# wenet-e2e/wesep

Hardware: AMD Instinct MI355X
Metric: utterances/sec (4 s, 16 kHz, 2-spk) fwd+bwd, pBSRNN (higher is better)
Workload: dtype bf16x3+fp16x2+fp16x1 split products (+fp8 lo terms), fp32 accumulate; 1 GPU; pBSRNN FiLM multi-fuse, 6 repeats, feature_dim 128, fixed 256-d embeddings; fwd + SI-SDR + bwd + per-tensor clip + Adam-L2; bf16x3 (x-projections, projections, d(hcat), BN / mask GEMMs) + fp16x2 (recurrent products of all four recurrence kernels, d(xn)) + fp16x1 (LSTM weight gradients); 2-byte saved gates / d(gates); fp32 accumulate; BPTT kernels: W_hh as fp16 hi + block-scaled FP8 lo; the lo term; rows_per_gpu=32, global_rows=32, samples_per_row=64000, parallelism=dp1

## Files before the change

wesep_amd/csrc/gemm_blk.hip:

```cpp
#include <stdlib.h>

#include <type_traits>

#include "common.h"

typedef __bf16 bf16x8 __attribute__((ext_vector_type(8)));
typedef unsigned int u32x4 __attribute__((ext_vector_type(4)));
typedef unsigned int u32x2 __attribute__((ext_vector_type(2)));
typedef float f32x2 __attribute__((ext_vector_type(2)));
typedef _Float16 f16x8 __attribute__((ext_vector_type(8)));
typedef _Float16 f16x2 __attribute__((ext_vector_type(2)));
typedef int i32x4 __attribute__((ext_vector_type(4)));
typedef int v8i __attribute__((ext_vector_type(8)));
typedef __fp16 h16x2 __attribute__((ext_vector_type(2)));

__device__ __forceinline__ f32x16 mfma32(bf16x8 a, bf16x8 b, f32x16 c) {
  return __builtin_amdgcn_mfma_f32_32x32x16_bf16(a, b, c, 0, 0, 0);
}

__device__ __forceinline__ void split8(const float* v, bf16x8& hi, bf16x8& lo) {
#pragma unroll
  for (int j = 0; j < 8; ++j) {
    hi[j] = (__bf16)v[j];
    lo[j] = (__bf16)(v[j] - (float)hi[j]);
// ... 365 lines not shown
    const int sc = __builtin_amdgcn_readfirstlane(sc_n);
    v8i a8;
#pragma unroll
    for (int hs = 0; hs < HS; ++hs) {
    acell ac[2 * KH];
#pragma unroll
    for (int q = 0; q < 2 * KH; ++q) ac[q] = an[q];
    if (hs == 0 && st + 1 < nstage) {
      wstage(st + 1, cur ^ 1);
      if constexpr (A16 == 3) sc_n = wsc[st + 1];
    }
    if (hs + 1 < HS) load_a(st, hs + 1);
    else if (st + 1 < nstage) load_a(st + 1, 0);
#pragma unroll
    for (int ksl = 0; ksl < KH; ++ksl) {
      const int ks = hs * KH + ksl;
      bf16x8 ah, al;
      if constexpr (A16 == 1) {
        const u32x2 c0 = __builtin_bit_cast(u32x2, ac[2 * ksl]), c1 = __builtin_bit_cast(u32x2, ac[2 * ksl + 1]);
        ah = __builtin_bit_cast(bf16x8, u32x4{c0[0], c0[1], c1[0], c1[1]});
      } else if constexpr (A16 == 3) {
        const u32x2 c0 = __builtin_bit_cast(u32x2, ac[2 * ksl]), c1 = __builtin_bit_cast(u32x2, ac[2 * ksl + 1]);
        const f16x8 a16 = __builtin_bit_cast(f16x8, u32x4{c0[0], c0[1], c1[0], c1[1]});
        typedef short s16x2 __attribute__((ext_vector_type(2)));
#pragma unroll
        for (int h2 = 0; h2 < 2; ++h2) {
          s16x2 c = {0, 0};
          c = __builtin_amdgcn_cvt_scalef32_pk_fp8_f16(c, f16x2{a16[4 * h2], a16[4 * h2 + 1]}, 256.f, false);
          c = __builtin_amdgcn_cvt_scalef32_pk_fp8_f16(c, f16x2{a16[4 * h2 + 2], a16[4 * h2 + 3]}, 256.f, true);
          a8[2 * ks + h2] = __builtin_bit_cast(int, c);
        }
        const u32x4* wt = &wl[cur][ks * 256 + lane];
#pragma unroll
        for (int nt = 0; nt < 4; ++nt)
          acc[nt] = __builtin_amdgcn_mfma_f32_32x32x16_f16(a16, __builtin_bit_cast(f16x8, wt[nt * 64]), acc[nt], 0, 0, 0);
        if (ks == 3) {
          const u32x4* w8 = &wl[cur][1024 + lane];
          auto frag = [&](int nt) {
            return __builtin_shufflevector(__builtin_bit_cast(i32x4, w8[(2 * nt) * 64]), __builtin_bit_cast(i32x4, w8[(2 * nt + 1) * 64]),
                                           0, 1, 2, 3, 4, 5, 6, 7);
          };
          acc[0] = __builtin_amdgcn_mfma_scale_f32_32x32x64_f8f6f4(a8, frag(0), acc[0], 0, 0, 0, 127 + 8, 0, sc);
          acc[1] = __builtin_amdgcn_mfma_scale_f32_32x32x64_f8f6f4(a8, frag(1), acc[1], 0, 0, 0, 127 + 8, 1, sc);
          acc[2] = __builtin_amdgcn_mfma_scale_f32_32x32x64_f8f6f4(a8, frag(2), acc[2], 0, 0, 0, 127 + 8, 2, sc);
          acc[3] = __builtin_amdgcn_mfma_scale_f32_32x32x64_f8f6f4(a8, frag(3), acc[3], 0, 0, 0, 127 + 8, 3, sc);
        }
        continue;
      } else if constexpr (A16 == 2) {
        const u32x2 c0 = __builtin_bit_cast(u32x2, ac[2 * ksl]), c1 = __builtin_bit_cast(u32x2, ac[2 * ksl + 1]);
        const f16x8 a16 = __builtin_bit_cast(f16x8, u32x4{c0[0], c0[1], c1[0], c1[1]});
        const u32x4* wt = &wl[cur][ks * 512 + lane];
#pragma unroll
        for (int nt = 0; nt < 4; ++nt) {
          acc[nt] = __builtin_amdgcn_mfma_f32_32x32x16_f16(a16, __builtin_bit_cast(f16x8, wt[(nt * 2) * 64]), acc[nt], 0, 0, 0);
          acc[nt] = __builtin_amdgcn_mfma_f32_32x32x16_f16(a16, __builtin_bit_cast(f16x8, wt[(nt * 2 + 1) * 64]), acc[nt], 0, 0, 0);
        }
        continue;
      } else {
        unpack8(__builtin_bit_cast(u32x4, ac[2 * ksl]), __builtin_bit_cast(u32x4, ac[2 * ksl + 1]), ah, al);
        if (p.a16_out && active) {
          unsigned short* o16 = reinterpret_cast<unsigned short*>(p.a16_out) + (long long)bb * 32 * K + i * 4 +
                                (long long)(st * 16 + 4 * ks + 2 * half) * 128;
#pragma unroll
          for (int c = 0; c < 2; ++c) {
            const u32x4 cell = __builtin_bit_cast(u32x4, ac[2 * ksl + c]);
            _Float16 h[4];
#pragma unroll
            for (int j = 0; j < 4; ++j)
              h[j] = (_Float16)(__uint_as_float(cell[j] & 0xffff0000u) + __uint_as_float(cell[j] << 16));
            const f16x2 p0 = {h[0], h[1]}, p1 = {h[2], h[3]};
            *reinterpret_cast<u32x2*>(o16 + c * 128) = u32x2{__builtin_bit_cast(unsigned, p0), __builtin_bit_cast(unsigned, p1)};
          }
        }
      }
      const u32x4* wt = &wl[cur][ks * 512 + lane];
#pragma unroll
      for (int nt = 0; nt < 4; ++nt) {
        const bf16x8 bh = __builtin_bit_cast(bf16x8, wt[(nt * 2) * 64]);
        const bf16x8 bl = __builtin_bit_cast(bf16x8, wt[(nt * 2 + 1) * 64]);
        acc[nt] = mfma32(ah, bh, acc[nt]);
        if constexpr (A16 != 1) acc[nt] = mfma32(al, bh, acc[nt]);
        acc[nt] = mfma32(ah, bl, acc[nt]);
      }
    }
    }
    asm volatile("s_waitcnt vmcnt(0)" ::: "memory");
    __syncthreads();
  }

  float* stg = reinterpret_cast<float*>(&wl[0][0]) + w * 2048;
#pragma unroll
  for (int pass = 0; pass < 2; ++pass) {
#pragma unroll
    for (int t = 0; t < 2; ++t) {
      const int nt = 2 * pass + t;
      const float bv = p.bias ? p.bias[nt * 32 + i] : 0.f;
#pragma unroll
      for (int r = 0; r < 16; ++r) {
        const int m = (r & 3) + 8 * (r >> 2) + 4 * half;
        stg[m * 64 + t * 32 + i] = (A16 >= 2 ? acc[nt][r] * inv_s : acc[nt][r]) + bv;
      }
    }
    __syncthreads();
    const int c4 = lane & 15, r0 = lane >> 4;
    f32x4 v[8];
    long long off[8];
#pragma unroll
    for (int k = 0; k < 8; ++k) {
      const int m = r0 + 4 * k;
      const long long pos = posl[w][m];
      off[k] = (active && pos >= 0) ? pos * p.ldc + pass * 64 + 4 * c4 : -1;
      v[k] = *reinterpret_cast<const f32x4*>(stg + m * 64 + 4 * c4);
    }
    if (p.R) {
#pragma unroll
      for (int k = 0; k < 8; ++k)
        if (off[k] >= 0) v[k] += *reinterpret_cast<const f32x4*>(p.R + off[k]);
    }
#pragma unroll
    for (int k = 0; k < 8; ++k)
      if (off[k] >= 0) *reinterpret_cast<f32x4*>(p.C + off[k]) = v[k];
    __syncthreads();
  }
}

extern "C" int ws_gemm_b2p(const ws_gemm_b2p_args* a, void* stream) {
  WS_REQUIRE(a && a->A && a->Wpack && a->C, "ws_gemm_b2p: null pointer");
  WS_REQUIRE(a->N == 128, "ws_gemm_b2p: N must be 128 (got %d)", a->N);
  WS_REQUIRE(a->a_fmt >= 0 && a->a_fmt <= 3 && (a->a_fmt < 2 || a->amax), "ws_gemm_b2p: a_fmt %d (2 / 3 need amax)", a->a_fmt);
  WS_REQUIRE(a->a_fmt == 0 || !a->a16_out, "ws_gemm_b2p: a16_out goes with a_fmt 0 (got a_fmt %d)", a->a_fmt);
  WS_REQUIRE(a->K > 0 && a->K % 64 == 0, "ws_gemm_b2p: K %% 64 (K=%d)", a->K);
  WS_REQUIRE(a->ldc >= a->N && a->ldc % 4 == 0, "ws_gemm_b2p: ldc >= N and ldc %% 4 == 0 (16-byte row pieces)");
  WS_REQUIRE(a->sm.nseq > 0 && a->sm.L > 0 && a->sm.sq_div > 0, "ws_gemm_b2p: bad sequence map");
  const int nblk = ((a->sm.nseq + 31) / 32) * a->sm.L;
  hipStream_t s = (hipStream_t)stream;
  ws_prof_begin(WS_PROF_GEMM_NT, s);
  if (a->a_fmt == 3)
    hipLaunchKernelGGL(gemm_b2p_kernel<3>, dim3((nblk + 7) / 8), dim3(512), 0, s, *a);
  else if (a->a_fmt == 2)
    hipLaunchKernelGGL(gemm_b2p_kernel<2>, dim3((nblk + 7) / 8), dim3(512), 0, s, *a);
  else if (a->a_fmt == 1)
    hipLaunchKernelGGL(gemm_b2p_kernel<1>, dim3((nblk + 7) / 8), dim3(512), 0, s, *a);
  else
    hipLaunchKernelGGL(gemm_b2p_kernel<0>, dim3((nblk + 7) / 8), dim3(512), 0, s, *a);
  ws_prof_end(WS_PROF_GEMM_NT, s);
  return ws_check_launch("ws_gemm_b2p");
}

typedef __bf16 bf16x4 __attribute__((ext_vector_type(4)));
#define TB_LD 40

typedef __bf16 bf16x2 __attribute__((ext_vector_type(2)));

template <int TA, bool ASUM>
__global__ __launch_bounds__(512, 2) void gemm_tnb_kernel(const ws_gemm_tnb_args p) {
  constexpr int NCOL = 128 * (1 + TA);
  constexpr int PLANE = NCOL * TB_LD;
  constexpr int NG = (1 + TA) / 2;
  constexpr int TN = TA == 1 ? 1 : TA;
  __shared__ __attribute__((aligned(16))) __bf16 ldsA[2 * PLANE];
  __shared__ __attribute__((aligned(16))) __bf16 ldsB[2 * PLANE];
  const int tid = threadIdx.x, lane = tid & 63, l31 = lane & 31, half = lane >> 5;
  const int w = __builtin_amdgcn_readfirstlane(tid >> 6);
  const int wm = w >> 2, wn = w & 3;
  const int gt = blockIdx.y, split = blockIdx.x;
  const int L = p.L;
  const int b_begin = split * p.blocks_per_split;
  const int b_end = min(p.nblk, b_begin + p.blocks_per_split);

  const float* gbase[NG];
  long long gstride[NG];
  int gshift[NG], gcol[NG];
#pragma unroll
  for (int r = 0; r < NG; ++r) {
    const int g = tid + 512 * r;
    const int part = g >> 8, quad = (g >> 3) & 31, sg = g & 7;
    gcol[r] = part * 128 + 4 * quad;
    if (part == 0) {
      gbase[r] = p.G + (long long)((p.g_off + gt * 128) / 4 + quad) * 128 + sg * 16;
      gstride[r] = 32LL * p.g_width;
      gshift[r] = 0;
    } else {
      const int c0 = (part - 1) * 128;
      const bool s1 = c0 >= p.a0_cols;
      const float* base = s1 ? p.A1 : p.A0;
      const int off = s1 ? p.a1_off + c0 - p.a0_cols : p.a0_off + c0;
      gbase[r] = base + (long long)(off / 4 + quad) * 128 + sg * 16;
      gstride[r] = 32LL * (s1 ? p.a1_width : p.a0_width);
      gshift[r] = s1 ? p.a1_shift : p.a0_shift;
    }
  }
  const int sg = tid & 7;

  f32x4 rq[2][NG][4];
  bool use[2][NG];
  auto load_block = [&](int b, int slot) {
    const int tile = b / L, step = b - tile * L;
#pragma unroll
    for (int r = 0; r < NG; ++r) {
      const int sa = step + gshift[r];
      use[slot][r] = sa >= 0 && sa < L;
      const float* src = gbase[r] + (long long)(use[slot][r] ? b + gshift[r] : b) * gstride[r];
#pragma unroll
      for (int j = 0; j < 4; ++j) rq[slot][r][j] = *reinterpret_cast<const f32x4*>(src + 4 * j);
    }
  };
  float csum[NG][4];
#pragma unroll
  for (int r = 0; r < NG; ++r)
#pragma unroll
    for (int c = 0; c < 4; ++c) csum[r][c] = 0.f;
  auto store_piece = [&](int slot, __bf16* lds, unsigned live, int pc) {
    const int r = pc >> 2, c = pc & 3;
    unsigned e[4];
#pragma unroll
    for (int j = 0; j < 4; ++j) {
      const float f = rq[slot][r][j][c];
      e[j] = __float_as_uint(f);
    }
    if (r > 0) {
      const unsigned m = use[slot][r] ? 0xffffffffu : 0u;
#pragma unroll
      for (int j = 0; j < 4; ++j) e[j] &= m;
    }
    if (r == 0 || ASUM) {
      const bf16x2 ones = __builtin_bit_cast(bf16x2, live);
#pragma unroll
      for (int j = 0; j < 4; ++j)
        csum[r][c] = __builtin_amdgcn_fdot2_f32_bf16(__builtin_bit_cast(bf16x2, e[j]), ones, csum[r][c], false);
    }
    uint2 hi, lo;
    hi.x = __builtin_amdgcn_perm(e[1], e[0], WS_SEL_HI16);
    hi.y = __builtin_amdgcn_perm(e[3], e[2], WS_SEL_HI16);
    lo.x = __builtin_amdgcn_perm(e[1], e[0], WS_SEL_LO16);
    lo.y = __builtin_amdgcn_perm(e[3], e[2], WS_SEL_LO16);
    const int o = (gcol[r] + c) * TB_LD + 4 * sg;
    *reinterpret_cast<uint2*>(lds + o) = hi;
    *reinterpret_cast<uint2*>(lds + PLANE + o) = lo;
  };
  auto store_block = [&](int slot, __bf16* lds, unsigned live) {
#pragma unroll
    for (int pc = 0; pc < 4 * NG; ++pc) store_piece(slot, lds, live, pc);
  };

  f32x16 acc[2][TN];
#pragma unroll
  for (int e = 0; e < 2; ++e)
#pragma unroll
    for (int f = 0; f < TN; ++f)
#pragma unroll
      for (int r = 0; r < 16; ++r) acc[e][f][r] = 0.f;

  const int nb = b_end - b_begin;
  if (nb > 0) {
    load_block(b_begin, 0);
    load_block(min(b_begin + 1, b_end - 1), 1);
    store_block(0, ldsA, 0x3f803f80u);
  }
  __syncthreads();
  for (int ib = 0; ib < nb; ib += 2) {
#pragma unroll
    for (int s = 0; s < 2; ++s) {
      const int i = ib + s;
      if (i < nb) {
        load_block(b_begin + min(i + 2, nb - 1), s);
        __builtin_amdgcn_sched_barrier(0);
        const __bf16* lds = s ? ldsB : ldsA;
        __bf16* ldsw = s ? ldsA : ldsB;
        const unsigned live = i + 1 < nb ? 0x3f803f80u : 0u;
        constexpr int NSUB = 6 * TN, NPC = 4 * NG, EVERY = NSUB / NPC;
        auto lda = [&](int ks, int f, bf16x8& h, bf16x8& l) {
          const int ra = (128 + wn * 32 * TN + f * 32 + l31) * TB_LD + ks + 8 * half;
          h = *reinterpret_cast<const bf16x8*>(lds + ra);
          l = *reinterpret_cast<const bf16x8*>(lds + PLANE + ra);
        };
        bf16x8 ah, al, ahn, aln;
        lda(0, 0, ah, al);
        int sub = 0;
#pragma unroll
        for (int ks = 0; ks < 32; ks += 16) {
          bf16x8 gh[2], gl[2];
#pragma unroll
          for (int e = 0; e < 2; ++e) {
            const int rg = (wm * 64 + e * 32 + l31) * TB_LD + ks + 8 * half;
            gh[e] = *reinterpret_cast<const bf16x8*>(lds + rg);
            gl[e] = *reinterpret_cast<const bf16x8*>(lds + PLANE + rg);
          }
#pragma unroll
          for (int f = 0; f < TN; ++f) {
            const bool last = ks == 16 && f == TN - 1;
#pragma unroll
            for (int term = 0; term < 3; ++term, ++sub) {
              if (term == 0 && !last) lda(f + 1 < TN ? ks : 16, f + 1 < TN ? f + 1 : 0, ahn, aln);
#pragma unroll
              for (int e = 0; e < 2; ++e)
                acc[e][f] = mfma32(term == 1 ? gl[e] : gh[e], term == 2 ? al : ah, acc[e][f]);
              if (sub % EVERY == 0 && sub / EVERY < NPC) store_piece(s ^ 1, ldsw, live, sub / EVERY);
              __builtin_amdgcn_sched_barrier(0);
            }
            ah = ahn; al = aln;
          }
        }
        __syncthreads();
      }
    }
  }

  const int ncols = p.a0_cols + p.a1_cols;
  float* out = p.slab + (long long)split * p.slab_stride;
#pragma unroll
  for (int e = 0; e < 2; ++e)
#pragma unroll
    for (int f = 0; f < TN; ++f) {
      const int acol = wn * 32 * TN + f * 32 + l31;
      if (acol < ncols) {
#pragma unroll
        for (int r = 0; r < 16; ++r) {
          const int grow = gt * 128 + wm * 64 + e * 32 + (r & 3) + 8 * (r >> 2) + 4 * half;
          out[(long long)grow * ncols + acol] = acc[e][f][r];
        }
      }
    }
#pragma unroll
  for (int r = 0; r < NG; ++r) {
    const int part = (tid + 512 * r) >> 8;
    float* dst = part == 0 ? p.bslab : (gt == 0 && (r == 0 || ASUM) ? p.aslab : nullptr);
#pragma unroll
    for (int c = 0; c < 4; ++c) {
      float t = csum[r][c];
      t += __shfl_xor(t, 1, 64);
      t += __shfl_xor(t, 2, 64);
      t += __shfl_xor(t, 4, 64);
      if (dst && sg == 0) {
        if (part == 0)
          dst[(long long)split * p.bslab_stride + gt * 128 + gcol[r] + c] = t;
        else
          dst[(long long)split * p.aslab_stride + gcol[r] - 128 + c] = t;
      }
    }
  }
}


template <bool ASUM, int GFMT, int GD, int AF = 0>
__global__ __launch_bounds__(512, 2) void gemm_tnb16_kernel(const ws_gemm_tnb_args p) {
  static_assert(AF == 0 || (GFMT == 3 && !ASUM), "fp16 A operand: scaled-fp16 G on the fp16 instruction, no column sums of A");
  constexpr int TA = 3, TN = 3;
  constexpr bool F16 = GFMT == 3;
  constexpr int NTERM = AF ? 1 : (GFMT == 2 ? 3 : 2);
  const float inv_s = GFMT >= 2 ? ws_dgates_scale_inv(*p.amax) : 1.f;
  const float inv_out = (F16 && !AF) ? inv_s * 0.015625f : inv_s;
  constexpr int NCOL = 128 * (1 + TA);
  constexpr int PLANE = NCOL * TB_LD;
  __shared__ __attribute__((aligned(16))) __bf16 ldsA[(AF ? 1 : 2) * PLANE];
  __shared__ __attribute__((aligned(16))) __bf16 ldsB[(AF ? 1 : 2) * PLANE];
  const int tid = threadIdx.x, lane = tid & 63, l31 = lane & 31, half = lane >> 5;
  const int w = __builtin_amdgcn_readfirstlane(tid >> 6);
  const int wm = w >> 2, wn = w & 3;
  const int gt = blockIdx.y, split = blockIdx.x;
  const int L = p.L;
  const int b_begin = split * p.blocks_per_split;
  const int b_end = min(p.nblk, b_begin + p.blocks_per_split);

  const int qg = tid >> 4, sp = tid & 15;
  const unsigned short* gsrc = reinterpret_cast<const unsigned short*>(p.G) +
                               ((long long)((p.g_off + gt * 128) / 4 + qg) * 32 + 2 * sp) * 4;
  const long long gstep = 32LL * p.g_width;
  const float* abase[2];
  long long astride[2];
  int ashift[2], acol[2], aslot[2];
#pragma unroll
  for (int r = 0; r < 2; ++r) {
    const int g = r == 0 ? tid : 512 + (tid >> 1);
    const int tile = g >> 8, quad = (g >> 3) & 31, sg = g & 7;
    const int c0 = tile * 128;
    const bool s1 = c0 >= p.a0_cols;
    const float* base = s1 ? p.A1 : p.A0;
    const int off = s1 ? p.a1_off + c0 - p.a0_cols : p.a0_off + c0;
    aslot[r] = 4 * sg + (r == 1 ? 2 * (tid & 1) : 0);
    abase[r] = AF ? reinterpret_cast<const float*>(reinterpret_cast<const unsigned short*>(base) +
                                                   (long long)(off / 4 + quad) * 128 + aslot[r] * 4)
                  : base + (long long)(off / 4 + quad) * 128 + aslot[r] * 4;
    astride[r] = 32LL * (s1 ? p.a1_width : p.a0_width);
    ashift[r] = s1 ? p.a1_shift : p.a0_shift;
    acol[r] = 128 + c0 + 4 * quad;
  }

  u32x4 gq[GD];
  f32x4 aq[2][AF ? 3 : 6];
  bool use[2][2];
  auto load_g = [&](int b, int gslot) { gq[gslot] = *reinterpret_cast<const u32x4*>(gsrc + (long long)b * gstep); };
  auto load_block = [&](int b, int slot) {
    const int tile = b / L, step = b - tile * L;
#pragma unroll
    for (int r = 0; r < 2; ++r) {
      const int sa = step + ashift[r];
      use[slot][r] = sa >= 0 && sa < L;
      if constexpr (AF) {
        const unsigned short* src = reinterpret_cast<const unsigned short*>(abase[r]) +
                                    (long long)(use[slot][r] ? b + ashift[r] : b) * astride[r];
#pragma unroll
        for (int j = 0; j < (r == 0 ? 2 : 1); ++j) aq[slot][2 * r + j] = *reinterpret_cast<const f32x4*>(src + 8 * j);
      } else {
        const float* src = abase[r] + (long long)(use[slot][r] ? b + ashift[r] : b) * astride[r];
#pragma unroll
        for (int j = 0; j < (r == 0 ? 4 : 2); ++j) aq[slot][4 * r + j] = *reinterpret_cast<const f32x4*>(src + 4 * j);
      }
    }
  };
  float gsum[4] = {0.f, 0.f, 0.f, 0.f}, asum[2][4];
#pragma unroll
  for (int r = 0; r < 2; ++r)
#pragma unroll
    for (int c = 0; c < 4; ++c) asum[r][c] = 0.f;
  auto store_piece = [&](int slot, int gslot, __bf16* lds, unsigned live, int pc) {
    const bf16x2 ones = __builtin_bit_cast(bf16x2, live);
    if (pc >= 8) {
      const u32x4 d = gq[gslot];
      const unsigned lo_ = pc == 8 ? d[0] : d[1], hi_ = pc == 8 ? d[2] : d[3];
      const int col = 4 * qg + 2 * (pc - 8);
      if constexpr (F16) {
        const unsigned c_even = __builtin_amdgcn_perm(hi_, lo_, WS_SEL_LO16), c_odd = __builtin_amdgcn_perm(hi_, lo_, WS_SEL_HI16);
        *reinterpret_cast<unsigned*>(lds + col * TB_LD + 2 * sp) = c_even;
        *reinterpret_cast<unsigned*>(lds + (col + 1) * TB_LD + 2 * sp) = c_odd;
        const h16x2 ones_h = __builtin_bit_cast(h16x2, live ? 0x3c003c00u : 0u);
        gsum[2 * (pc - 8)] = __builtin_amdgcn_fdot2(__builtin_bit_cast(h16x2, c_even), ones_h, gsum[2 * (pc - 8)], false);
        gsum[2 * (pc - 8) + 1] = __builtin_amdgcn_fdot2(__builtin_bit_cast(h16x2, c_odd), ones_h, gsum[2 * (pc - 8) + 1], false);
        return;
      }
      if constexpr (GFMT == 2) {
        const f16x2 a = __builtin_bit_cast(f16x2, lo_), b = __builtin_bit_cast(f16x2, hi_);
        const float x[4] = {(float)a[0], (float)a[1], (float)b[0], (float)b[1]};
        __bf16 h[4], l[4];
#pragma unroll
        for (int j = 0; j < 4; ++j) {
          h[j] = (__bf16)x[j];
          l[j] = (__bf16)(x[j] - (float)h[j]);
        }
        const bf16x2 he = {h[0], h[2]}, ho = {h[1], h[3]}, le = {l[0], l[2]}, lodd = {l[1], l[3]};
        *reinterpret_cast<bf16x2*>(lds + col * TB_LD + 2 * sp) = he;
        *reinterpret_cast<bf16x2*>(lds + (col + 1) * TB_LD + 2 * sp) = ho;
        *reinterpret_cast<bf16x2*>(lds + PLANE + col * TB_LD + 2 * sp) = le;
        *reinterpret_cast<bf16x2*>(lds + PLANE + (col + 1) * TB_LD + 2 * sp) = lodd;
        if (live) {
          gsum[2 * (pc - 8)] += x[0] + x[2];
          gsum[2 * (pc - 8) + 1] += x[1] + x[3];
        }
        return;
      }
      const unsigned c_even = __builtin_amdgcn_perm(hi_, lo_, WS_SEL_LO16), c_odd = __builtin_amdgcn_perm(hi_, lo_, WS_SEL_HI16);
      *reinterpret_cast<unsigned*>(lds + col * TB_LD + 2 * sp) = c_even;
      *reinterpret_cast<unsigned*>(lds + (col + 1) * TB_LD + 2 * sp) = c_odd;
      gsum[2 * (pc - 8)] = __builtin_amdgcn_fdot2_f32_bf16(__builtin_bit_cast(bf16x2, c_even), ones, gsum[2 * (pc - 8)], false);
      gsum[2 * (pc - 8) + 1] =
          __builtin_amdgcn_fdot2_f32_bf16(__builtin_bit_cast(bf16x2, c_odd), ones, gsum[2 * (pc - 8) + 1], false);
      return;
    }
    const int r = pc >> 2, c = pc & 3;
    const unsigned m = use[slot][r] ? 0xffffffffu : 0u;
    if constexpr (AF) {
      const unsigned sel = (c & 1) ? WS_SEL_HI16 : WS_SEL_LO16;
      const int wi = c >> 1;
      const u32x4 q0 = __builtin_bit_cast(u32x4, aq[slot][2 * r]);
      const unsigned x = __builtin_amdgcn_perm(q0[2 + wi], q0[wi], sel) & m;
      const int o = (acol[r] + c) * TB_LD + aslot[r];
      if (r == 0) {
        const u32x4 q1 = __builtin_bit_cast(u32x4, aq[slot][1]);
        const unsigned y = __builtin_amdgcn_perm(q1[2 + wi], q1[wi], sel) & m;
        *reinterpret_cast<uint2*>(lds + o) = uint2{x, y};
      } else {
        *reinterpret_cast<unsigned*>(lds + o) = x;
      }
      return;
    }
    unsigned e[4];
#pragma unroll
    for (int j = 0; j < (r == 0 ? 4 : 2); ++j) {
      const float f = aq[slot][4 * r + j][c];
      e[j] = __float_as_uint(f) & m;
    }
    if (ASUM) {
#pragma unroll
      for (int j = 0; j < (r == 0 ? 4 : 2); ++j)
        asum[r][c] = __builtin_amdgcn_fdot2_f32_bf16(__builtin_bit_cast(bf16x2, e[j]), ones, asum[r][c], false);
    }
    const int o = (acol[r] + c) * TB_LD + aslot[r];
    if constexpr (F16) {
      unsigned hw[2], lw[2];
#pragma unroll
      for (int j = 0; j < (r == 0 ? 2 : 1); ++j) {
        const unsigned u0 = e[2 * j] + 0x03000300u, u1 = e[2 * j + 1] + 0x03000300u;
        hw[j] = __builtin_bit_cast(unsigned, __builtin_amdgcn_cvt_pkrtz(__uint_as_float(u0 & 0xffff0000u), __uint_as_float(u1 & 0xffff0000u)));
        lw[j] = __builtin_bit_cast(unsigned, __builtin_amdgcn_cvt_pkrtz(__uint_as_float(u0 << 16), __uint_as_float(u1 << 16)));
      }
      if (r == 0) {
        *reinterpret_cast<uint2*>(lds + o) = uint2{hw[0], hw[1]};
        *reinterpret_cast<uint2*>(lds + PLANE + o) = uint2{lw[0], lw[1]};
      } else {
        *reinterpret_cast<unsigned*>(lds + o) = hw[0];
        *reinterpret_cast<unsigned*>(lds + PLANE + o) = lw[0];
      }
      return;
    }
    if (r == 0) {
      uint2 hi, lo;
      hi.x = __builtin_amdgcn_perm(e[1], e[0], WS_SEL_HI16);
      hi.y = __builtin_amdgcn_perm(e[3], e[2], WS_SEL_HI16);
      lo.x = __builtin_amdgcn_perm(e[1], e[0], WS_SEL_LO16);
      lo.y = __builtin_amdgcn_perm(e[3], e[2], WS_SEL_LO16);
      *reinterpret_cast<uint2*>(lds + o) = hi;
      *reinterpret_cast<uint2*>(lds + PLANE + o) = lo;
    } else {
      *reinterpret_cast<unsigned*>(lds + o) = __builtin_amdgcn_perm(e[1], e[0], WS_SEL_HI16);
      *reinterpret_cast<unsigned*>(lds + PLANE + o) = __builtin_amdgcn_perm(e[1], e[0], WS_SEL_LO16);
    }
  };
  constexpr int NPC = 10;
  auto store_block = [&](int slot, int gslot, __bf16* lds, unsigned live) {
#pragma unroll
    for (int pc = 0; pc < NPC; ++pc) store_piece(slot, gslot, lds, live, pc);
  };

  f32x16 acc[2][TN];
#pragma unroll
  for (int e = 0; e < 2; ++e)
#pragma unroll
    for (int f = 0; f < TN; ++f)
#pragma unroll
      for (int r = 0; r < 16; ++r) acc[e][f][r] = 0.f;

  const int nb = b_end - b_begin;
  if (nb > 0) {
    load_block(b_begin, 0);
    load_block(min(b_begin + 1, b_end - 1), 1);
#pragma unroll
    for (int k = 0; k < GD; ++k) load_g(min(b_begin + k, b_end - 1), k);
    store_block(0, 0, ldsA, 0x3f803f80u);
  }
  __syncthreads();
  for (int ib = 0; ib < nb; ib += GD) {
#pragma unroll
    for (int sg4 = 0; sg4 < GD; ++sg4) {
      const int s = sg4 & 1;
      const int i = ib + sg4;
      if (i < nb) {
        load_block(b_begin + min(i + 2, nb - 1), s);
        load_g(b_begin + min(i + GD, nb - 1), sg4);
        __builtin_amdgcn_sched_barrier(0);
        const __bf16* lds = s ? ldsB : ldsA;
        __bf16* ldsw = s ? ldsA : ldsB;
        const unsigned live = i + 1 < nb ? 0x3f803f80u : 0u;
        auto lda = [&](int ks, int f, bf16x8& h, bf16x8& l) {
          const int ra = (128 + wn * 32 * TN + f * 32 + l31) * TB_LD + ks + 8 * half;
          h = *reinterpret_cast<const bf16x8*>(lds + ra);
          if constexpr (!AF) l = *reinterpret_cast<const bf16x8*>(lds + PLANE + ra);
        };
        bf16x8 ah, al, ahn, aln;
        lda(0, 0, ah, al);
        int sub = 0;
#pragma unroll
        for (int ks = 0; ks < 32; ks += 16) {
          bf16x8 gh[2], gl[2];
#pragma unroll
          for (int e = 0; e < 2; ++e) {
            gh[e] = *reinterpret_cast<const bf16x8*>(lds + (wm * 64 + e * 32 + l31) * TB_LD + ks + 8 * half);
            if constexpr (GFMT == 2) gl[e] = *reinterpret_cast<const bf16x8*>(lds + PLANE + (wm * 64 + e * 32 + l31) * TB_LD + ks + 8 * half);
          }
#pragma unroll
          for (int f = 0; f < TN; ++f) {
            const bool last = ks == 16 && f == TN - 1;
#pragma unroll
            for (int term = 0; term < NTERM; ++term, ++sub) {
              if (term == 0 && !last) lda(f + 1 < TN ? ks : 16, f + 1 < TN ? f + 1 : 0, ahn, aln);
#pragma unroll
              for (int e = 0; e < 2; ++e) {
                if constexpr (F16)
                  acc[e][f] = __builtin_amdgcn_mfma_f32_32x32x16_f16(__builtin_bit_cast(f16x8, gh[e]),
                                                                     __builtin_bit_cast(f16x8, term == 1 ? al : ah), acc[e][f], 0, 0, 0);
                else
                  acc[e][f] = mfma32(term == 2 ? gl[e] : gh[e], term == 1 ? al : ah, acc[e][f]);
              }
              if constexpr (NTERM == 1) {
                if (2 * sub < NPC) store_piece(s ^ 1, (sg4 + 1) % GD, ldsw, live, 2 * sub);
                if (2 * sub + 1 < NPC) store_piece(s ^ 1, (sg4 + 1) % GD, ldsw, live, 2 * sub + 1);
              } else if (sub < NPC) {
                store_piece(s ^ 1, (sg4 + 1) % GD, ldsw, live, sub);
              }
              __builtin_amdgcn_sched_barrier(0);
            }
            ah = ahn; al = aln;
          }
        }
        __syncthreads();
      }
    }
  }

  const int ncols = p.a0_cols + p.a1_cols;
  float* out = p.slab + (long long)split * p.slab_stride;
#pragma unroll
  for (int e = 0; e < 2; ++e)
#pragma unroll
    for (int f = 0; f < TN; ++f) {
      const int ac_ = wn * 32 * TN + f * 32 + l31;
      if (ac_ < ncols) {
#pragma unroll
        for (int r = 0; r < 16; ++r) {
          const int grow = gt * 128 + wm * 64 + e * 32 + (r & 3) + 8 * (r >> 2) + 4 * half;
          out[(long long)grow * ncols + ac_] = GFMT >= 2 ? acc[e][f][r] * inv_out : acc[e][f][r];
        }
      }
    }
#pragma unroll
  for (int c = 0; c < 4; ++c) {
    float t = gsum[c];
    t += __shfl_xor(t, 1, 64);
    t += __shfl_xor(t, 2, 64);
    t += __shfl_xor(t, 4, 64);
    t += __shfl_xor(t, 8, 64);
    if (p.bslab && sp == 0) p.bslab[(long long)split * p.bslab_stride + gt * 128 + 4 * qg + c] = GFMT >= 2 ? t * inv_s : t;
  }
  if (ASUM && gt == 0 && p.aslab) {
#pragma unroll
    for (int r = 0; r < 2; ++r)
#pragma unroll
      for (int c = 0; c < 4; ++c) {
        float t = asum[r][c];
        t += __shfl_xor(t, 1, 64);
        t += __shfl_xor(t, 2, 64);
        t += __shfl_xor(t, 4, 64);
        if (r == 1) t += __shfl_xor(t, 8, 64);
        const bool first = r == 0 ? (tid & 7) == 0 : (tid & 15) == 0;
        if (first) p.aslab[(long long)split * p.aslab_stride + acol[r] - 128 + c] = t;
      }
  }
}

extern "C" int ws_gemm_tnb(const ws_gemm_tnb_args* a, void* stream) {
  WS_REQUIRE(a && a->G && a->A0 && a->slab, "ws_gemm_tnb: null pointer");
  WS_REQUIRE(a->g_cols > 0 && a->g_cols % 128 == 0 && a->g_off % 4 == 0 && a->g_width % 4 == 0,
             "ws_gemm_tnb: G column range");
  WS_REQUIRE(a->a0_cols > 0 && a->a0_cols % 128 == 0 && a->a0_off % 4 == 0 && a->a0_width % 4 == 0,
             "ws_gemm_tnb: A0 column range");
  WS_REQUIRE(a->a1_cols == 0 || (a->A1 && a->a1_cols % 128 == 0 && a->a1_off % 4 == 0 && a->a1_width % 4 == 0),
             "ws_gemm_tnb: A1 column range");
  const int ta = (a->a0_cols + a->a1_cols) / 128;
  WS_REQUIRE(ta == 1 || ta == 3, "ws_gemm_tnb: A columns must total 128 or 384 (got %d)", ta * 128);
  WS_REQUIRE(a->a0_shift == 0, "ws_gemm_tnb: only A1 can be shifted (a0_shift = %d)", a->a0_shift);
  WS_REQUIRE(a->g_fmt == 0 || ((a->g_fmt == 1 || a->g_fmt == 2) && ta == 3),
             "ws_gemm_tnb: g_fmt 1 / 2 (2-byte G) are built for 384 A columns");
  WS_REQUIRE(a->g_fmt != 2 || a->amax, "ws_gemm_tnb: g_fmt = 2 (scaled fp16 G) needs amax");
  WS_REQUIRE(a->a_fmt == 0 || (a->a_fmt == 1 && a->g_fmt == 2 && !a->aslab && ta == 3),
             "ws_gemm_tnb: a_fmt = 1 (fp16 A operands) is built for g_fmt = 2, 384 A columns, no aslab");
  WS_REQUIRE(a->nblk > 0 && a->L > 0 && a->nblk % a->L == 0 && a->nsplit > 0 && a->blocks_per_split > 0 &&
                 (long long)a->nsplit * a->blocks_per_split >= a->nblk,
             "ws_gemm_tnb: bad block split");
  hipStream_t s = (hipStream_t)stream;
  dim3 grid(a->nsplit, a->g_cols / 128), block(512);
  ws_prof_begin(WS_PROF_GEMM_TN, s);
  static const int gdepth = [] { const char* e = getenv("WS_TNB_GDEPTH"); return e && atoi(e) == 2 ? 2 : 4; }();
  const char* f16env = getenv("WS_TNB_F16");
  const bool f16mm = !(f16env && atoi(f16env) == 0);
  if (a->a_fmt == 1)
    hipLaunchKernelGGL((gemm_tnb16_kernel<false, 3, 4, 1>), grid, block, 0, s, *a);
  else if (a->g_fmt == 2 && f16mm && a->aslab)
    hipLaunchKernelGGL((gemm_tnb16_kernel<true, 3, 4>), grid, block, 0, s, *a);
  else if (a->g_fmt == 2 && f16mm)
    hipLaunchKernelGGL((gemm_tnb16_kernel<false, 3, 4>), grid, block, 0, s, *a);
  else if (a->g_fmt == 2 && a->aslab)
    hipLaunchKernelGGL((gemm_tnb16_kernel<true, 2, 4>), grid, block, 0, s, *a);
  else if (a->g_fmt == 2 && gdepth == 2)
    hipLaunchKernelGGL((gemm_tnb16_kernel<false, 2, 2>), grid, block, 0, s, *a);
  else if (a->g_fmt == 2)
    hipLaunchKernelGGL((gemm_tnb16_kernel<false, 2, 4>), grid, block, 0, s, *a);
  else if (a->g_fmt && a->aslab)
    hipLaunchKernelGGL((gemm_tnb16_kernel<true, 1, 4>), grid, block, 0, s, *a);
  else if (a->g_fmt && gdepth == 2)
    hipLaunchKernelGGL((gemm_tnb16_kernel<false, 1, 2>), grid, block, 0, s, *a);
  else if (a->g_fmt)
    hipLaunchKernelGGL((gemm_tnb16_kernel<false, 1, 4>), grid, block, 0, s, *a);
  else if (ta == 3 && a->aslab)
    hipLaunchKernelGGL((gemm_tnb_kernel<3, true>), grid, block, 0, s, *a);
  else if (ta == 3)
    hipLaunchKernelGGL((gemm_tnb_kernel<3, false>), grid, block, 0, s, *a);
  else
    hipLaunchKernelGGL((gemm_tnb_kernel<1, true>), grid, block, 0, s, *a);
  ws_prof_end(WS_PROF_GEMM_TN, s);
  return ws_check_launch("ws_gemm_tnb");
}
```

wesep_amd/dev.py:

```python
import ctypes as C
import os
from typing import NamedTuple, Optional

import numpy as np
import torch

from . import _lib as L

BIG = 1 << 30


def gemm_mode() -> str:
    return os.environ.get("WESEP_GEMM", "bf16x3")


def _mode_bit(mode):
    return 4 if (mode or gemm_mode()) == "bf16x3" else 0
GN_EPS = float(np.finfo(np.float32).eps)


class Rows(NamedTuple):
    div: int
    s1: int
    s2: int
# ... 732 lines not shown
    L.check(L.lib().ws_debug_occupy(nblocks, usec, _word(stop), None, L.stream_ptr()), "ws_debug_occupy")


def prof_enable(on: bool):
    L.check(L.lib().ws_prof_enable(int(on)), "ws_prof_enable")


def prof_collect(kind: int):
    ms = C.c_double(0.0)
    n = C.c_longlong(0)
    L.check(L.lib().ws_prof_collect(kind, C.byref(ms), C.byref(n)), "ws_prof_collect")
    return ms.value, n.value


def bl_num_blocks(sm: SeqMap) -> int:
    return -(-sm.nseq // 32) * sm.L


def bl_positions(sm: SeqMap, device):
    ntile = -(-sm.nseq // 32)
    seq = torch.arange(ntile * 32, device=device).view(ntile, 1, 32)
    step = torch.arange(sm.L, device=device).view(1, sm.L, 1)
    nv = sm.nvalid or sm.nseq
    valid = (seq < nv).expand(ntile, sm.L, 32)
    sq = seq.clamp(max=nv - 1)
    pos = torch.div(sq, sm.div, rounding_mode="floor") * sm.s1 + (sq % sm.div) * sm.s2 + step * sm.step_rows
    return (pos * valid).reshape(-1), valid.reshape(-1)


def bls_pack(x: torch.Tensor) -> torch.Tensor:
    hi = x.to(torch.bfloat16)
    lo = (x - hi.float()).to(torch.bfloat16)
    bits = (hi.view(torch.int16).to(torch.int32) << 16) | (lo.view(torch.int16).to(torch.int32) & 0xffff)
    return bits.view(torch.float32)


def bls_unpack(x: torch.Tensor) -> torch.Tensor:
    bits = x.contiguous().view(torch.int32)
    return (bits & -65536).view(torch.float32) + (bits << 16).view(torch.float32)


def to_blocked(x: torch.Tensor, sm: SeqMap, split=False) -> torch.Tensor:
    pos, valid = bl_positions(sm, x.device)
    C_ = x.shape[1]
    rows = x[pos] * valid[:, None].to(x.dtype)
    out = rows.view(-1, 32, C_ // 4, 4).permute(0, 2, 1, 3).contiguous()
    return bls_pack(out) if split else out


def from_blocked(xb: torch.Tensor, sm: SeqMap, P: int, split=False) -> torch.Tensor:
    if split:
        xb = bls_unpack(xb)
    pos, valid = bl_positions(sm, xb.device)
    nblk, Cq = xb.shape[0], xb.shape[1]
    rows = xb.permute(0, 2, 1, 3).reshape(nblk * 32, Cq * 4)
    out = torch.zeros(P, Cq * 4, device=xb.device, dtype=xb.dtype)
    out[pos[valid]] = rows[valid]
    return out


def blh_bf16_pack(xb: torch.Tensor) -> torch.Tensor:
    return xb.to(torch.bfloat16).contiguous().view(torch.float32)


def blh_f16_pack(xb: torch.Tensor) -> torch.Tensor:
    return xb.to(torch.float16).contiguous().view(torch.float32)


def blh_f16_unpack(buf: torch.Tensor, nblk: int, C_: int) -> torch.Tensor:
    return buf.reshape(-1)[: nblk * 32 * C_ // 2].view(torch.float16).view(nblk, C_ // 4, 32, 4).float()


def blh_bf16_unpack(buf: torch.Tensor, nblk: int, C_: int) -> torch.Tensor:
    return buf.reshape(-1)[: nblk * 32 * C_ // 2].view(torch.bfloat16).view(nblk, C_ // 4, 32, 4).float()


def blh_gates_unpack(buf: torch.Tensor, nblk: int) -> torch.Tensor:
    Cq = 2 * 4 * L.LSTM_H // 4
    code = (buf.reshape(-1)[: nblk * 32 * Cq * 2].view(torch.int16).to(torch.int32) & 0xFFFF).view(nblk, Cq, 32, 4).double()
    s_sig = float(torch.tensor(1.0 / 65535.0, dtype=torch.float32))
    s_tanh = float(torch.tensor(1.0 / 32767.5, dtype=torch.float32))
    is_g = ((torch.arange(Cq, device=buf.device) >> 6) & 3 == 2).view(1, Cq, 1, 1)
    return torch.where(is_g, code * s_tanh - 1.0, code * s_sig).float()


def _smc(sm: SeqMap):
    c = L.SeqMapC()
    c.sq_s1, c.sq_s2, c.step_rows, c.nseq, c.sq_div, c.L = sm.s1, sm.s2, sm.step_rows, sm.nseq, sm.div, sm.L
    c.nvalid = sm.nvalid
    return c


def pack_w(W, N: int, K: int, ldw: int, out, trans=False, order=0, w_off=0, f16=False):
    _chk(W, "W")
    _chk(out, "out")
    if out.numel() < N * K:
        raise L.WesepHipError("pack_w: output too small")
    if int(f16) == 2:
        if order != 1:
            raise L.WesepHipError("pack_w: the fp16 + FP8 pack exists in the b2p order only")
        L.check(L.lib().ws_pack_w_f16f8(_p(W, w_off), N, K, ldw, int(trans), _p(out), L.stream_ptr()), "ws_pack_w_f16f8")
        return
    fn = L.lib().ws_pack_w_f16 if f16 else L.lib().ws_pack_w
    L.check(fn(_p(W, w_off), N, K, ldw, int(trans), order, _p(out), L.stream_ptr()), "ws_pack_w_f16" if f16 else "ws_pack_w")


def gemm_p2b(*, A, lda: int, sm: SeqMap, Wpack, N: int, C_out, K=128, bias=None, A_bl=None, stats=None,
             gamma=None, beta=None, stat_map: Optional[StatMap] = None, run_if=None, amax=None, A_bl16=None, steps=None,
             steps_div=1):
    for n, t in (("A", A), ("Wpack", Wpack), ("bias", bias), ("C", C_out), ("A_bl", A_bl), ("stats", stats),
                 ("gamma", gamma), ("beta", beta), ("A_bl16", A_bl16)):
        _chk(t, n)
    a = L.GemmP2BArgs()
    a.A, a.Wpack, a.bias, a.C, a.A_bl = _p(A), _p(Wpack), _p(bias), _p(C_out), _p(A_bl)
    a.stats, a.gamma, a.beta = _p(stats), _p(gamma), _p(beta)
    a.sm = _smc(sm)
    st = stat_map or StatMap(1, 0, 1, 0, 0)
    a.st_div1, a.st_m1, a.st_div2, a.st_m2, a.st_base = st
    a.lda, a.N, a.K = lda, N, K
    a.run_if = C.c_void_p(run_if.data_ptr()) if run_if is not None else None
    a.amax = C.c_void_p(amax.data_ptr()) if amax is not None else None
    a.A_bl16 = _p(A_bl16)
    if ALG is not None and run_if is None:
        rows = (getattr(sm, "nvalid", 0) or sm.nseq) * sm.L
        _alg("gemm_nt", rows * (4 * K + 4 * N + (4 * K if A_bl is not None else 0) + (2 * K if A_bl16 is not None else 0)) + 4 * N * K,
             2 * rows * N * K)
    if steps is not None:
        _chk_lens(steps, -(-(getattr(sm, "nvalid", 0) or sm.nseq) // steps_div), "ws_gemm_p2b_len")
        L.check(L.lib().ws_gemm_p2b_len(C.byref(a), _tab(steps), steps_div, L.stream_ptr()), "ws_gemm_p2b_len")
        return
    L.check(L.lib().ws_gemm_p2b(C.byref(a), L.stream_ptr()), "ws_gemm_p2b")


def gemm_b2p(*, A, K: int, sm: SeqMap, Wpack, C_out, ldc: int, N=128, bias=None, R=None, a_fmt=0, amax=None, a16_out=None):
    for n, t in (("A", A), ("Wpack", Wpack), ("bias", bias), ("C", C_out), ("R", R), ("a16_out", a16_out)):
        _chk(t, n)
    if a16_out is not None and a_fmt != 0:
        raise L.WesepHipError("gemm_b2p: a16_out goes with a_fmt = 0 (split-pair A)")
    a = L.GemmB2PArgs()
    a.A, a.Wpack, a.bias, a.R, a.C = _p(A), _p(Wpack), _p(bias), _p(R), _p(C_out)
    a.sm = _smc(sm)
    a.ldc, a.N, a.K, a.a_fmt = ldc, N, K, a_fmt
    a.amax = C.c_void_p(amax.data_ptr()) if amax is not None else None
    a.a16_out = _p(a16_out)
    if ALG is not None:
        rows = (getattr(sm, "nvalid", 0) or sm.nseq) * sm.L
        _alg("gemm_nt", rows * ((2 if a_fmt else 4) * K + 4 * N * (1 + (R is not None)) + (2 * K if a16_out is not None else 0))
             + 4 * N * K, 2 * rows * N * K)
    L.check(L.lib().ws_gemm_b2p(C.byref(a), L.stream_ptr()), "ws_gemm_b2p")


def tnb_splits(nblk: int, gtiles: int):
    cap = int(os.environ.get("WESEP_TNB_MAXSPLIT", "64"))
    nsplit = max(1, min(cap, int(os.environ.get("WESEP_TNB_WGS", "256")) // gtiles, nblk))
    if nsplit >= 8:
        nsplit -= nsplit % 8
    bps = -(-nblk // nsplit)
    return nsplit, bps


def gemm_tnb(*, G, g_width: int, g_off: int, g_cols: int, A0, a0_width: int, a0_off: int, a0_cols: int,
             nblk: int, L_: int, slab, nsplit: int, blocks_per_split: int, a0_shift=0, A1=None, a1_width=0,
             a1_off=0, a1_cols=0, a1_shift=0, bslab=None, aslab=None, g_fmt=0, amax=None, a_fmt=0):
    for n, t in (("G", G), ("A0", A0), ("A1", A1), ("slab", slab), ("bslab", bslab), ("aslab", aslab)):
        _chk(t, n)
    a = L.GemmTNBArgs()
    a.G, a.A0, a.A1, a.slab, a.bslab, a.aslab = _p(G), _p(A0), _p(A1), _p(slab), _p(bslab), _p(aslab)
    a.slab_stride = g_cols * (a0_cols + a1_cols)
    a.bslab_stride = g_cols
    a.aslab_stride = a0_cols + a1_cols
    a.g_width, a.g_off, a.g_cols = g_width, g_off, g_cols
    a.a0_width, a.a0_off, a.a0_cols, a.a0_shift = a0_width, a0_off, a0_cols, a0_shift
    a.a1_width, a.a1_off, a.a1_cols, a.a1_shift = a1_width, a1_off, a1_cols, a1_shift
    a.nblk, a.L, a.nsplit, a.blocks_per_split, a.g_fmt, a.a_fmt = nblk, L_, nsplit, blocks_per_split, g_fmt, a_fmt
    a.amax = C.c_void_p(amax.data_ptr()) if amax is not None else None
    if ALG is not None:
        rows, acols = nblk * 32, a0_cols + a1_cols
        _alg("gemm_tn", rows * ((2 if g_fmt else 4) * g_cols + (2 if a_fmt else 4) * acols) + 4 * nsplit * g_cols * acols,
             2 * rows * g_cols * acols)
    L.check(L.lib().ws_gemm_tnb(C.byref(a), L.stream_ptr()), "ws_gemm_tnb")


LN_EPS = 1e-5


def _call(name, *args):
    L.check(getattr(L.lib(), name)(*args, L.stream_ptr()), name)


def flat_stats(x, ngroups: int, n_per_group: int, stats, eps=LN_EPS, nchunk=None):
    if nchunk is None:
        nchunk = max(1, min(max(1, 512 // ngroups), n_per_group // 16384))
    scratch = torch.empty(ngroups, nchunk, 4, device=x.device, dtype=torch.float32)
    for n, t in (("x", x), ("stats", stats)):
        _chk(t, n)
    _call("ws_flat_stats", _p(x), ngroups, n_per_group, eps, nchunk, _p(scratch), _p(stats))


def prelu_fwd(x, rb, a, rows: int, Cc: int, rows_per_r: int, y):
    for n, t in (("x", x), ("rb", rb), ("a", a), ("y", y)):
        _chk(t, n)
    _call("ws_prelu_fwd", _p(x), _p(rb), _p(a), rows, Cc, rows_per_r, _p(y))


def prelu_bwd(pre, dy, a, dx):
    for n, t in (("pre", pre), ("dy", dy), ("a", a), ("dx", dx)):
        _chk(t, n)
    n = pre.numel()
    nslab = max(1, min(1024, n // 4096))
    slab = torch.empty(nslab, device=pre.device, dtype=torch.float32)
    _call("ws_prelu_bwd", _p(pre), _p(dy), _p(a), n, _p(dx), _p(slab), nslab)
    da = torch.empty(1, device=pre.device, dtype=torch.float32)
    reduce_slabs(slab, nslab, 1, 1, da)
    return da


def dwconv_fwd(x, stats, gamma, beta, w, b, R: int, Tp: int, Cc: int, P: int, dil: int, st_div: int, y, causal=False):
    for n, t in (("x", x), ("stats", stats), ("gamma", gamma), ("beta", beta), ("w", w), ("b", b), ("y", y)):
        _chk(t, n)
    _call("ws_dwconv_ex_fwd", _p(x), _p(stats), _p(gamma), _p(beta), _p(w), _p(b), R, Tp, Cc, P, dil, st_div, int(causal),
          _p(y))


def row_splits(M: int, target=1024):
    nsplit = max(1, min(target, M // 64))
    rows = -(-M // nsplit)
    return -(-M // rows), rows


def dwconv_bwd(dy, x, stats, gamma, beta, w, R: int, Tp: int, Cc: int, P: int, dil: int, st_div: int, dxn, causal=False):
    for n, t in (("dy", dy), ("x", x), ("stats", stats), ("gamma", gamma), ("beta", beta), ("w", w), ("dxn", dxn)):
        _chk(t, n)
    nsplit, rows = row_splits(R * Tp)
    slab = torch.empty(nsplit, P + 1, Cc, device=dy.device, dtype=torch.float32)
    _call("ws_dwconv_ex_bwd", _p(dy), _p(x), _p(stats), _p(gamma), _p(beta), _p(w), R, Tp, Cc, P, dil, st_div,
          int(causal), _p(dxn), nsplit, rows, _p(slab))
    out = torch.empty(P + 1, Cc, device=dy.device, dtype=torch.float32)
    reduce_slabs(slab, nsplit, (P + 1) * Cc, (P + 1) * Cc, out)
    return out[:P].t().contiguous(), out[P].contiguous()


def chan_sums(g, x, stats, st_div: int, rows_per_group: int, ngroups: int, Cc: int):
    for n, t in (("g", g), ("x", x), ("stats", stats)):
        _chk(t, n)
    nsplit = max(1, min(max(1, 1024 // ngroups), rows_per_group // 32))
    slab = torch.empty(nsplit, ngroups, 2, Cc, device=g.device, dtype=torch.float32)
    _call("ws_chan_sums", _p(g), _p(x), _p(stats), st_div, rows_per_group, ngroups, nsplit, Cc, _p(slab))
    out = torch.empty(ngroups, 2, Cc, device=g.device, dtype=torch.float32)
    reduce_slabs(slab, nsplit, ngroups * 2 * Cc, ngroups * 2 * Cc, out)
    return out


def norm_ab(sums, gamma, ngroups: int, Cc: int, n_per_group: int, ab):
    for n, t in (("sums", sums), ("gamma", gamma), ("ab", ab)):
        _chk(t, n)
    _call("ws_norm_ab", _p(sums), _p(gamma), ngroups, Cc, n_per_group, _p(ab))


def norm_bwd_apply_cl(x, dxn, stats, ab, gamma, res, rows: int, Cc: int, st_div: int, dx):
    for n, t in (("x", x), ("dxn", dxn), ("stats", stats), ("ab", ab), ("gamma", gamma), ("res", res), ("dx", dx)):
        _chk(t, n)
    _call("ws_norm_bwd_apply_cl", _p(x), _p(dxn), _p(stats), _p(ab), _p(gamma), _p(res), rows, Cc, st_div, _p(dx))


def maskmul_fwd(w, w_off: int, ldw: int, m, rows: int, N: int, s):
    for n, t in (("w", w), ("m", m), ("s", s)):
        _chk(t, n)
    _call("ws_maskmul_fwd", _p(w, w_off), ldw, _p(m), rows, N, _p(s))


def maskmul_bwd(ds, w, w_off: int, ldw: int, m, rows: int, N: int, dw, dw_off: int, ld_dw: int, dm):
    for n, t in (("ds", ds), ("w", w), ("m", m), ("dw", dw), ("dm", dm)):
        _chk(t, n)
    _call("ws_maskmul_bwd", _p(ds), _p(w, w_off), ldw, _p(m), rows, N, _p(dw, dw_off), ld_dw, _p(dm))


def relu_mask(d, y):
    for n, t in (("d", d), ("y", y)):
        _chk(t, n)
    _call("ws_relu_mask", _p(d), _p(y), d.numel())


def ola_fwd(frames, bias, R: int, Tp: int, Lk: int, hop: int, Tout: int, est):
    for n, t in (("frames", frames), ("bias", bias), ("est", est)):
        _chk(t, n)
    _call("ws_ola_fwd", _p(frames), _p(bias), R, Tp, Lk, hop, Tout, _p(est))


def ola_bwd(dest, R: int, Tp: int, Lk: int, hop: int, Tout: int, dframes):
    for n, t in (("dest", dest), ("dframes", dframes)):
        _chk(t, n)
    _call("ws_ola_bwd", _p(dest), R, Tp, Lk, hop, Tout, _p(dframes))


def total_sum(x):
    _chk(x, "x")
    n = x.numel()
    nslab = max(1, min(1024, n // 4096))
    slab = torch.empty(nslab, device=x.device, dtype=torch.float32)
    _call("ws_sum_partial", _p(x), n, _p(slab), nslab)
    out = torch.empty(1, device=x.device, dtype=torch.float32)
    reduce_slabs(slab, nslab, 1, 1, out)
    return out


BN_EPS, BN_MOMENTUM = 1e-5, 0.1

# ... 929 lines not shown
```

Measured before the change: 341.4 utterances/s.

## Stage two K-blocks per barrier in fp16-A weight-gradient TN GEMM

Adds an SB=2 variant of the fp16-A (a_fmt==1) TN-block gradient GEMM. It keeps four single-plane LDS images, so the next block is written into LDS while the current one is consumed, and it calls __syncthreads only every second block. The loop is unrolled over the LCM of the register ring depths. This variant becomes the default for a_fmt==1, and the default split count halves (128 workgroups instead of 256) so each split covers more blocks. The cost is more LDS per workgroup (about 160 KB), which can lower occupancy, and fewer workgroups filling the GPU.

```diff
diff --git a/wesep_amd/csrc/gemm_blk.hip b/wesep_amd/csrc/gemm_blk.hip
--- a/wesep_amd/csrc/gemm_blk.hip
+++ b/wesep_amd/csrc/gemm_blk.hip
@@ -541,6 +541,9 @@
 
 typedef __bf16 bf16x2 __attribute__((ext_vector_type(2)));
 
+constexpr int tnb_gcd(int a, int b) { return b ? tnb_gcd(b, a % b) : a; }
+constexpr int tnb_lcm(int a, int b) { return a / tnb_gcd(a, b) * b; }
+
 template <int TA, bool ASUM>
 __global__ __launch_bounds__(512, 2) void gemm_tnb_kernel(const ws_gemm_tnb_args p) {
   constexpr int NCOL = 128 * (1 + TA);
@@ -731,7 +734,7 @@
 }
 
 
-template <bool ASUM, int GFMT, int GD, int AF = 0>
+template <bool ASUM, int GFMT, int GD, int AF = 0, int SB = 1>
 __global__ __launch_bounds__(512, 2) void gemm_tnb16_kernel(const ws_gemm_tnb_args p) {
   static_assert(AF == 0 || (GFMT == 3 && !ASUM), "fp16 A operand: scaled-fp16 G on the fp16 instruction, no column sums of A");
   constexpr int TA = 3, TN = 3;
@@ -743,6 +746,20 @@
   constexpr int PLANE = NCOL * TB_LD;
   __shared__ __attribute__((aligned(16))) __bf16 ldsA[(AF ? 1 : 2) * PLANE];
   __shared__ __attribute__((aligned(16))) __bf16 ldsB[(AF ? 1 : 2) * PLANE];
+  static_assert(SB == 1 || (SB == 2 && AF == 1), "two blocks per barrier: four one-plane images = 160 KB");
+  constexpr int AD = 2;
+  constexpr bool WT = SB == 2;
+  static_assert(GD >= 2, "ring depth");
+  constexpr int NIMG = 2 * SB;
+  __shared__ __attribute__((aligned(16))) __bf16 ldsC[SB == 2 ? PLANE : 8];
+  __shared__ __attribute__((aligned(16))) __bf16 ldsD[SB == 2 ? PLANE : 8];
+  auto image = [&](int k) -> __bf16* {
+    if constexpr (SB == 2) {
+      if (k == 2) return ldsC;
+      if (k == 3) return ldsD;
+    }
+    return k == 1 ? ldsB : ldsA;
+  };
   const int tid = threadIdx.x, lane = tid & 63, l31 = lane & 31, half = lane >> 5;
   const int w = __builtin_amdgcn_readfirstlane(tid >> 6);
   const int wm = w >> 2, wn = w & 3;
@@ -776,8 +793,8 @@
   }
 
   u32x4 gq[GD];
-  f32x4 aq[2][AF ? 3 : 6];
-  bool use[2][2];
+  f32x4 aq[AD][AF ? 3 : 6];
+  bool use[AD][2];
   auto load_g = [&](int b, int gslot) { gq[gslot] = *reinterpret_cast<const u32x4*>(gsrc + (long long)b * gstep); };
   auto load_block = [&](int b, int slot) {
     const int tile = b / L, step = b - tile * L;
@@ -920,68 +937,80 @@
 
   const int nb = b_end - b_begin;
   if (nb > 0) {
-    load_block(b_begin, 0);
-    load_block(min(b_begin + 1, b_end - 1), 1);
+#pragma unroll
+    for (int k = 0; k < AD; ++k) load_block(min(b_begin + k, b_end - 1), k);
 #pragma unroll
     for (int k = 0; k < GD; ++k) load_g(min(b_begin + k, b_end - 1), k);
-    store_block(0, 0, ldsA, 0x3f803f80u);
+#pragma unroll
+    for (int k = 0; k < SB; ++k) store_block(k, k, image(k), k < nb ? 0x3f803f80u : 0u);
+    if constexpr (SB == 2) {
+      load_block(b_begin + min(AD, nb - 1), 0);
+      load_g(b_begin + min(GD, nb - 1), 0);
+    }
   }
   __syncthreads();
-  for (int ib = 0; ib < nb; ib += GD) {
-#pragma unroll
-    for (int sg4 = 0; sg4 < GD; ++sg4) {
-      const int s = sg4 & 1;
-      const int i = ib + sg4;
-      if (i < nb) {
-        load_block(b_begin + min(i + 2, nb - 1), s);
-        load_g(b_begin + min(i + GD, nb - 1), sg4);
-        __builtin_amdgcn_sched_barrier(0);
-        const __bf16* lds = s ? ldsB : ldsA;
-        __bf16* ldsw = s ? ldsA : ldsB;
-        const unsigned live = i + 1 < nb ? 0x3f803f80u : 0u;
-        auto lda = [&](int ks, int f, bf16x8& h, bf16x8& l) {
-          const int ra = (128 + wn * 32 * TN + f * 32 + l31) * TB_LD + ks + 8 * half;
-          h = *reinterpret_cast<const bf16x8*>(lds + ra);
-          if constexpr (!AF) l = *reinterpret_cast<const bf16x8*>(lds + PLANE + ra);
-        };
-        bf16x8 ah, al, ahn, aln;
-        lda(0, 0, ah, al);
-        int sub = 0;
-#pragma unroll
-        for (int ks = 0; ks < 32; ks += 16) {
-          bf16x8 gh[2], gl[2];
+  constexpr int UN = tnb_lcm(tnb_lcm(AD, GD), NIMG);
+  auto step = [&](int i, int u) __attribute__((always_inline)) {
+    load_block(b_begin + min(i + SB - 1 + AD, nb - 1), (u + SB - 1) % AD);
+    load_g(b_begin + min(i + SB - 1 + GD, nb - 1), (u + SB - 1) % GD);
+    __builtin_amdgcn_sched_barrier(0);
+    const __bf16* lds = image(u % NIMG);
+    __bf16* ldsw = image((u + SB) % NIMG);
+    const unsigned live = i + SB < nb ? 0x3f803f80u : 0u;
+    auto lda = [&](int ks, int f, bf16x8& h, bf16x8& l) {
+      const int ra = (128 + wn * 32 * TN + f * 32 + l31) * TB_LD + ks + 8 * half;
+      h = *reinterpret_cast<const bf16x8*>(lds + ra);
+      if constexpr (!AF) l = *reinterpret_cast<const bf16x8*>(lds + PLANE + ra);
+    };
+    bf16x8 ah, al, ahn, aln;
+    lda(0, 0, ah, al);
+    int sub = 0;
+#pragma unroll
+    for (int ks = 0; ks < 32; ks += 16) {
+      bf16x8 gh[2], gl[2];
+#pragma unroll
+      for (int e = 0; e < 2; ++e) {
+        gh[e] = *reinterpret_cast<const bf16x8*>(lds + (wm * 64 + e * 32 + l31) * TB_LD + ks + 8 * half);
+        if constexpr (GFMT == 2) gl[e] = *reinterpret_cast<const bf16x8*>(lds + PLANE + (wm * 64 + e * 32 + l31) * TB_LD + ks + 8 * half);
+      }
+#pragma unroll
+      for (int f = 0; f < TN; ++f) {
+        const bool last = ks == 16 && f == TN - 1;
+#pragma unroll
+        for (int term = 0; term < NTERM; ++term, ++sub) {
+          if (term == 0 && !last) lda(f + 1 < TN ? ks : 16, f + 1 < TN ? f + 1 : 0, ahn, aln);
 #pragma unroll
           for (int e = 0; e < 2; ++e) {
-            gh[e] = *reinterpret_cast<const bf16x8*>(lds + (wm * 64 + e * 32 + l31) * TB_LD + ks + 8 * half);
-            if constexpr (GFMT == 2) gl[e] = *reinterpret_cast<const bf16x8*>(lds + PLANE + (wm * 64 + e * 32 + l31) * TB_LD + ks + 8 * half);
+            if constexpr (F16)
+              acc[e][f] = __builtin_amdgcn_mfma_f32_32x32x16_f16(__builtin_bit_cast(f16x8, gh[e]),
+                                                                 __builtin_bit_cast(f16x8, term == 1 ? al : ah), acc[e][f], 0, 0, 0);
+            else
+              acc[e][f] = mfma32(term == 2 ? gl[e] : gh[e], term == 1 ? al : ah, acc[e][f]);
           }
-#pragma unroll
-          for (int f = 0; f < TN; ++f) {
-            const bool last = ks == 16 && f == TN - 1;
-#pragma unroll
-            for (int term = 0; term < NTERM; ++term, ++sub) {
-              if (term == 0 && !last) lda(f + 1 < TN ? ks : 16, f + 1 < TN ? f + 1 : 0, ahn, aln);
-#pragma unroll
-              for (int e = 0; e < 2; ++e) {
-                if constexpr (F16)
-                  acc[e][f] = __builtin_amdgcn_mfma_f32_32x32x16_f16(__builtin_bit_cast(f16x8, gh[e]),
-                                                                     __builtin_bit_cast(f16x8, term == 1 ? al : ah), acc[e][f], 0, 0, 0);
-                else
-                  acc[e][f] = mfma32(term == 2 ? gl[e] : gh[e], term == 1 ? al : ah, acc[e][f]);
-              }
-              if constexpr (NTERM == 1) {
-                if (2 * sub < NPC) store_piece(s ^ 1, (sg4 + 1) % GD, ldsw, live, 2 * sub);
-                if (2 * sub + 1 < NPC) store_piece(s ^ 1, (sg4 + 1) % GD, ldsw, live, 2 * sub + 1);
-              } else if (sub < NPC) {
-                store_piece(s ^ 1, (sg4 + 1) % GD, ldsw, live, sub);
-              }
-              __builtin_amdgcn_sched_barrier(0);
-            }
-            ah = ahn; al = aln;
+          if constexpr (NTERM == 1) {
+            if (2 * sub < NPC) store_piece((u + SB) % AD, (u + SB) % GD, ldsw, live, 2 * sub);
+            if (2 * sub + 1 < NPC) store_piece((u + SB) % AD, (u + SB) % GD, ldsw, live, 2 * sub + 1);
+          } else if (sub < NPC) {
+            store_piece((u + SB) % AD, (u + SB) % GD, ldsw, live, sub);
           }
+          __builtin_amdgcn_sched_barrier(0);
         }
-        __syncthreads();
-      }
+        ah = ahn; al = aln;
+      }
+    }
+    if (SB == 1 || (u & 1)) __syncthreads();
+  };
+  int ib = 0;
+  if constexpr (WT) {
+    for (; ib + UN <= nb; ib += UN) {
+#pragma unroll
+      for (int u = 0; u < UN; ++u) step(ib + u, u);
+    }
+  }
+  for (; ib < nb; ib += UN) {
+#pragma unroll
+    for (int u = 0; u < UN; ++u) {
+      if (ib + u < nb) step(ib + u, u);
     }
   }
 
@@ -1023,6 +1052,10 @@
         if (first) p.aslab[(long long)split * p.aslab_stride + acol[r] - 128 + c] = t;
       }
   }
+}
+
+static void tnb16_a16_two_block_launch(dim3 grid, dim3 block, hipStream_t s, const ws_gemm_tnb_args& a) {
+  hipLaunchKernelGGL((gemm_tnb16_kernel<false, 3, 4, 1, 2>), grid, block, 0, s, a);
 }
 
 extern "C" int ws_gemm_tnb(const ws_gemm_tnb_args* a, void* stream) {
@@ -1050,7 +1083,10 @@
   static const int gdepth = [] { const char* e = getenv("WS_TNB_GDEPTH"); return e && atoi(e) == 2 ? 2 : 4; }();
   const char* f16env = getenv("WS_TNB_F16");
   const bool f16mm = !(f16env && atoi(f16env) == 0);
-  if (a->a_fmt == 1)
+  const char* pipeenv = getenv("WS_TNB_PIPE");
+  if (a->a_fmt == 1 && !(pipeenv && atoi(pipeenv) == 0))
+    tnb16_a16_two_block_launch(grid, block, s, *a);
+  else if (a->a_fmt == 1)
     hipLaunchKernelGGL((gemm_tnb16_kernel<false, 3, 4, 1>), grid, block, 0, s, *a);
   else if (a->g_fmt == 2 && f16mm && a->aslab)
     hipLaunchKernelGGL((gemm_tnb16_kernel<true, 3, 4>), grid, block, 0, s, *a);
diff --git a/wesep_amd/dev.py b/wesep_amd/dev.py
--- a/wesep_amd/dev.py
+++ b/wesep_amd/dev.py
@@ -908,7 +908,8 @@
 
 def tnb_splits(nblk: int, gtiles: int):
     cap = int(os.environ.get("WESEP_TNB_MAXSPLIT", "64"))
-    nsplit = max(1, min(cap, int(os.environ.get("WESEP_TNB_WGS", "256")) // gtiles, nblk))
+    wgs = "256" if os.environ.get("WS_TNB_PIPE", "").strip() == "0" else "128"
+    nsplit = max(1, min(cap, int(os.environ.get("WESEP_TNB_WGS", wgs)) // gtiles, nblk))
     if nsplit >= 8:
         nsplit -= nsplit % 8
     bps = -(-nblk // nsplit)
```

Result: no change. 343.6 utterances/s, median of 6 (+0.6%).
